# guofei-tju/MVML-MPI

Measured on AMD Instinct MI355X. Metric: molecules/sec GAT-view fwd+bwd at 1/2/4/8 GPU; % HBM peak on aggregation, higher is better.
Workload: dtype f32

## Files before the change

### include/mvml_gat.h

```cpp
#ifndef MVML_GAT_H
#define MVML_GAT_H

#include <stddef.h>
#include <stdint.h>

#ifdef __cplusplus
extern "C" {
#endif

#define MVML_OK 0
#define MVML_ERR_INVALID 1
#define MVML_ERR_LAUNCH 2
#define MVML_ERR_WORKSPACE 3

const char* mvml_last_error(void);
const char* mvml_version(void);

#define MVML_OPT_BIG_WINDOW 0
#define MVML_OPT_BWD_ATOMWISE 1
#define MVML_OPT_GEMM_TILE 2
#define MVML_OPT_GEMM_PERSIST 3
#define MVML_OPT_GEMM_NSPLIT 4
#define MVML_OPT_GEMM_RING 5
#define MVML_OPT_LSTM_TILE 6
// ... 118 lines not shown
                           int64_t ldgx, void* stream);
int mvml_gat_fold_weights(const float* fc_w, const float* res_fc_w, const float* attn_lr, int H,
                          int F, int Fin, int ldw, int mean_residual, float* Wcat, void* stream);
int mvml_gat_unfold_grads(const float* gWcat, const float* attn_lr, int H, int F, int Fin,
                          int ldg, int mean_residual, float* g_fc_w, float* g_res_fc_w,
                          void* stream);
size_t mvml_gat_proj_fwd_workspace_size(int64_t num_nodes, int H, int F);
int mvml_gat_proj_fwd(int64_t num_nodes, const float* X, int64_t ldx, int64_t K,
                      const float* Wcat, int64_t ldw, const float* attn_lr, int H, int F,
                      int mean_residual, int algo , float* Y, int64_t ldy,
                      float* elr, const uint32_t* amax_x, const uint32_t* amax_w,
                      const uint16_t* w_planes, int64_t w_plane, void* workspace,
                      size_t workspace_bytes, void* stream);
size_t mvml_gat_attn_grad_workspace_size(int64_t num_nodes, int H, int F);
int mvml_gat_attn_grad(int64_t num_nodes, int H, int F, const float* Y, int64_t ldy,
                       const float* gelr, int64_t ldgl, float* g_attn_l, float* g_attn_r,
                       void* workspace, size_t workspace_bytes, void* stream);
int mvml_gat_agg_fwd(int64_t num_nodes, const int32_t* node_groups, int64_t num_groups,
                     const int32_t* in_rowptr, const int32_t* in_src, const float* Y, int64_t ldy,
                     int H, int F, const float* elr, const float* bias, float slope, int mode,
                     float* out, float* attn, uint32_t* out_amax, uint32_t* out_row_amax,
                     void* stream);
int mvml_gat_agg_fwd_res(int64_t num_nodes, const int32_t* node_groups, int64_t num_groups,
                         const int32_t* in_rowptr, const int32_t* in_src, const float* Y,
                         int64_t ldy, int H, int F, const float* elr, const float* R, int64_t ldr,
                         const float* bias, float slope, int mode, float* out, float* attn,
                         uint32_t* out_amax, uint32_t* out_row_amax, void* stream);
size_t mvml_gat_agg_bwd_workspace_size(int64_t num_edges, int H);
int mvml_gat_agg_bwd(int64_t num_nodes, const int32_t* node_groups, int64_t num_groups,
                     const int32_t* in_rowptr, const int32_t* in_src, const int32_t* out_rowptr,
                     const int32_t* out_dst, const int32_t* out_inslot, const float* Y,
                     int64_t ldy, const float* elr, const float* attn, const float* out,
                     const float* g_out, int H, int F, float slope, int mode, float* gY,
                     int64_t ldgy, uint32_t* gy_amax, uint32_t* gy_row_amax, void* workspace,
                     size_t workspace_bytes, void* stream);
int mvml_gat_agg_bwd_res(int64_t num_nodes, const int32_t* node_groups, int64_t num_groups,
                         const int32_t* in_rowptr, const int32_t* in_src, const int32_t* out_rowptr,
                         const int32_t* out_dst, const int32_t* out_inslot, const float* Y,
                         int64_t ldy, const float* elr, const float* attn, const float* out,
                         const float* g_out, int H, int F, float slope, int mode, float* gY,
                         int64_t ldgy, int64_t elr_col, float* gR, int64_t ldgr, uint32_t* gy_amax,
                         uint32_t* gy_row_amax, void* workspace, size_t workspace_bytes, void* stream);
size_t mvml_gat_layer_bwd_workspace_size(int64_t num_nodes, int64_t num_edges, int H, int F, int Fin,
                                         int mean);
int mvml_gat_layer_bwd(int64_t num_nodes, const int32_t* node_groups, int64_t num_groups,
                       const int32_t* in_rowptr, const int32_t* in_src, const int32_t* out_rowptr,
                       const int32_t* out_dst, const int32_t* out_inslot, int64_t num_edges, int H,
                       int F, int Fin, int mean, float slope, const float* X, const float* Wcat,
                       const float* attn_lr, const float* Y, int64_t ldy, const float* elr,
                       const float* attn, const float* out, const float* g_out, float* g_X,
                       float* g_fc, float* g_res, float* g_attn, float* g_bias, void* workspace,
                       size_t workspace_bytes, void* stream);

int mvml_gatv2_agg_fwd(int64_t num_nodes, const int32_t* in_rowptr, const int32_t* in_src,
                       const float* ZL, int64_t ldzl, const float* ZR, int64_t ldzr, int H, int F,
                       const float* attn_vec, const float* R, int64_t ldr, float slope, int mode,
                       float* out, float* attn, void* stream);
int64_t mvml_gatv2_partial_rows(int64_t num_nodes);
size_t mvml_gatv2_agg_bwd_workspace_size(int64_t num_nodes, int64_t num_edges, int H, int F);
int mvml_gatv2_agg_bwd(int64_t num_nodes, const int32_t* in_rowptr, const int32_t* in_src,
                       const int32_t* out_rowptr, const int32_t* out_dst, const int32_t* out_inslot,
                       int64_t num_edges, const float* ZL, int64_t ldzl, const float* ZR,
                       int64_t ldzr, int H, int F, const float* attn_vec, const float* attn,
                       const float* out, const float* g_out, float slope, int mode, float* gZL,
                       int64_t ldgzl, float* gZR, int64_t ldgzr, float* gR, int64_t ldgr,
                       float* g_attn_vec, void* workspace, size_t workspace_bytes, void* stream);
int mvml_add_cols_f32(int64_t rows, int cols, const float* src, int64_t lds, float* dst, int64_t ldd,
                      void* stream);

int mvml_lstm_gates_cell_plan_ok(int64_t M, int D, int64_t K);
int mvml_lstm_gates_cell_fwd(int64_t M, int D, int64_t K, const float* A, int64_t lda,
                             const float* w_perm, int64_t ldw, const float* b_ih,
                             const float* b_hh, const float* c_prev, float* c_out, float* h_out,
                             int64_t ldh, float* act, float* h_out2, int64_t ldh2,
                             const uint32_t* amax_a, const uint32_t* amax_b ,
                             const uint32_t* amax_a_rows ,
                             const uint16_t* w_planes, int64_t w_plane ,
                             void* stream);
int mvml_segment_max_bits(int64_t B, const int64_t* node_offsets, const uint32_t* in_bits,
                          uint32_t floor_bits, uint32_t* out_bits, void* stream);
int mvml_lstm_cell_fwd(int64_t B, int D, const float* gates_pre, const float* b_ih,
                       const float* b_hh, const float* c_prev, float* c_out, float* h_out,
                       int64_t ldh, float* act_out, float* h_out2, int64_t ldh2, void* stream);
int64_t mvml_lstm_cell_bwd_part_rows(int64_t B, int D);
int mvml_lstm_cell_bwd(int64_t B, int D, const float* act, const float* c, const float* c_prev,
                       const float* g_h, int64_t ldgh, const float* g_h2, int64_t ldgh2,
                       const float* g_c, float* g_gates, float* g_c_prev, uint32_t* gg_amax,
                       float* gb_part, void* stream);
int mvml_set2set_seg_fwd(int64_t B, int D, const int64_t* node_offsets, const float* X,
                         float* qstar, int64_t ldq, float* lse, void* stream);
int mvml_set2set_seg_bwd(int64_t B, int D, const int64_t* node_offsets, const float* X,
                         const float* qstar, int64_t ldq, const float* lse,
                         const float* g_qstar, int64_t ldgq, float* g_q, int64_t ldgout,
                         float* alpha, float* g_e, void* stream);
int mvml_set2set_gx(int64_t num_nodes, int D, int T, const int32_t* node_graph,
                    const int64_t* node_offsets, int64_t num_graphs,
                    const float* qstars, int64_t ldq, int64_t qstar_stride,
                    const float* g_qstars, int64_t ldgq, int64_t g_qstar_stride,
                    const float* alphas, const float* g_es, float* gX, void* stream);

int mvml_wsum_max_fwd(int64_t B, int64_t N, int D, const int64_t* node_offsets, const float* X,
                      int64_t ldx, const float* W, const float* bias, float* out, int64_t ldo,
                      float* gate, int32_t* argmax, int64_t lda, void* stream);
int64_t mvml_wsum_max_bwd_part_rows(int64_t B);
int mvml_wsum_max_bwd(int64_t B, int64_t N, int D, const int64_t* node_offsets, const float* X,
                      int64_t ldx, const float* W, const float* gate, const int32_t* argmax,
                      int64_t lda, const float* g_out, int64_t ldgo, float* gX, int64_t ldgx,
                      float* part, int64_t ldp, void* stream);

int mvml_graphnorm_fwd(int64_t G, int D, const int64_t* group_offsets, const float* x,
                       const float* weight, const float* bias, const float* mean_scale,
                       float eps, float* y, void* stream);
size_t mvml_graphnorm_bwd_workspace_size(int64_t G, int D);
int mvml_graphnorm_bwd(int64_t G, int D, const int64_t* group_offsets, const float* x,
                       const float* weight, const float* mean_scale, float eps,
                       const float* g_y, float* g_x, float* g_weight, float* g_bias,
                       float* g_mean_scale, void* workspace, size_t workspace_bytes,
                       void* stream);

int64_t mvml_batchnorm1d_part_rows(int64_t M);
size_t mvml_batchnorm1d_workspace_size(int64_t M, int C);
int mvml_batchnorm1d_fwd(int64_t M, int C, const float* x, int64_t ldx, const float* weight,
                         const float* bias, int training, double momentum, double eps,
                         float* running_mean, float* running_var, int64_t* num_batches_tracked,
                         float* y, int64_t ldy, double* save_mean, double* save_invstd,
                         void* workspace, size_t workspace_bytes, void* stream);
int mvml_batchnorm1d_bwd(int64_t M, int C, const float* x, int64_t ldx, const float* weight,
                         int training, const double* save_mean, const double* save_invstd,
                         const float* g_y, int64_t ldgy, float* g_x, int64_t ldgx, float* g_weight,
                         float* g_bias, void* workspace, size_t workspace_bytes, void* stream);

int mvml_relu_bwd(int64_t n, const float* y, const float* g_y, float* g_x, float scale, void* stream);
int mvml_dropout_fwd(int64_t n, const float* x, float* y, double p, int64_t seed, void* stream);
int mvml_copy_cols(int64_t rows, int cols, const float* src, int64_t lds, float* dst, int64_t ldd,
                   void* stream);
int mvml_fill_zero(void* p, int64_t rows, int64_t row_bytes, int64_t pitch_bytes, void* stream);
int mvml_lstm_pack_weights(int D, int kin, const float* w_ih, const float* w_hh, float* wcat,
                           float* wperm, void* stream);
int mvml_transpose(int64_t rows, int64_t cols, const float* src, int64_t lds, float* dst, int64_t ldd,
                   void* stream);
int mvml_scale_by(int64_t n, const float* x, const float* s, float* y, void* stream);

int mvml_layernorm_fwd(int64_t rows, int D, const float* x, int64_t ldx, const float* gamma,
                       const float* beta, float eps, float* y, int64_t ldy, float* mean,
                       float* rstd, void* stream);
int mvml_layernorm_bwd(int64_t rows, int D, const float* x, int64_t ldx, const float* gamma,
                       const float* mean, const float* rstd, const float* g_y, int64_t ldgy,
                       float* g_x, int64_t ldgx, float* g_y_xhat, void* stream);
int mvml_token_attn_fwd(int64_t B, int H, int dk, const float* qkv, int64_t ld, float scale,
                        float* att, float* P, void* stream);
int mvml_token_attn_bwd(int64_t B, int H, int dk, const float* qkv, int64_t ld, float scale,
                        const float* P, const float* g_att, float* g_qkv, int64_t ldg,
                        void* stream);
int mvml_token_attn_fold_fwd(int64_t B, int H, int dk, const float* pv, int64_t ld,
                             const float* x, int64_t ldx, float scale, float* att, float* P,
                             void* stream);
int mvml_token_attn_fold_bwd(int64_t B, int H, int dk, const float* pv, int64_t ld,
                             const float* x, int64_t ldx, float scale, const float* P,
                             const float* g_att, float* g_pv, int64_t ldg, float* g_k,
                             int64_t ldgk, uint32_t* g_pv_amax, void* stream);
int mvml_conv3_fwd(int64_t B, int C, int O, int W, const float* in, const float* weight,
                   const float* bias, float* out, void* stream);
size_t mvml_conv3_bwd_workspace_size(int64_t B);
int mvml_conv3_bwd(int64_t B, int C, int O, int W, const float* in, const float* weight,
                   const float* out, const float* g_out, float* g_in, float* g_weight,
                   float* g_bias, void* workspace, size_t workspace_bytes, void* stream);
// ... 92 lines not shown
```

### mvml-mpi_amd/csrc/capi.cpp

```cpp
#include <stdarg.h>
#include <stdio.h>
#include <stdlib.h>

#include <atomic>

#include "common.h"

namespace mvml {

static thread_local char g_err[512] = {0};

void set_error(const char* fmt, ...) {
  va_list ap;
  va_start(ap, fmt);
  vsnprintf(g_err, sizeof(g_err), fmt, ap);
  va_end(ap);
}

void clear_error() { g_err[0] = 0; }

int check_launch(const char* what) {
  hipError_t e = hipGetLastError();
  if (e != hipSuccess) {
    set_error("%s: %s", what, hipGetErrorString(e));
    return MVML_ERR_LAUNCH;
  }
  return MVML_OK;
}

constexpr int kOptCount = 12;
static std::atomic<int> g_opt[kOptCount];
static int env_int(const char* name, int dflt) {
  const char* e = getenv(name);
  return e ? atoi(e) : dflt;
}
static const bool g_opt_init = [] {
  g_opt[MVML_OPT_BIG_WINDOW] = env_int("MVML_BIG_WINDOW", 1);
  g_opt[MVML_OPT_BWD_ATOMWISE] = env_int("MVML_BWD_ATOMWISE", 0);
  g_opt[MVML_OPT_GEMM_TILE] = env_int("MVML_X3_TILE", 0);
  g_opt[MVML_OPT_GEMM_PERSIST] = env_int("MVML_X3W_PERSIST", 256);
  g_opt[MVML_OPT_GEMM_NSPLIT] = env_int("MVML_GEMM_NSPLIT", 1);
  g_opt[MVML_OPT_GEMM_RING] = env_int("MVML_GEMM_RING", 0);
  g_opt[MVML_OPT_LSTM_TILE] = env_int("MVML_LSTM_TILE", 0);
  g_opt[MVML_OPT_MEAN_SRC] = env_int("MVML_MEAN_SRC", 1);
  g_opt[MVML_OPT_FLAT_SRC] = env_int("MVML_FLAT_SRC", 0);
  g_opt[MVML_OPT_DST_FWD] = env_int("MVML_DST_FWD", 0);
  g_opt[MVML_OPT_DST_UNR] = env_int("MVML_DST_UNR", 0);
  g_opt[MVML_OPT_SMALLK] = env_int("MVML_SMALLK", 1);
  return true;
}();

int option(int i) { return g_opt[i].load(std::memory_order_relaxed); }

}

extern "C" int mvml_set_option(int opt, int value) {
  if (opt < 0 || opt >= mvml::kOptCount) return -1;
  return mvml::g_opt[opt].exchange(value, std::memory_order_relaxed);
}

extern "C" int mvml_get_option(int opt) {
  if (opt < 0 || opt >= mvml::kOptCount) return -1;
  return mvml::option(opt);
}

extern "C" const char* mvml_last_error(void) { return mvml::g_err; }

extern "C" const char* mvml_version(void) { return "mvml_gat 0.1.0 (gfx950)"; }
```

### mvml-mpi_amd/csrc/set2set.hip

```cpp
#include <numeric>

#include "common.h"
#include "wave_ops.h"

namespace mvml {
namespace {

__device__ __forceinline__ float sigm(float x) { return 1.f / (1.f + expf(-x)); }

__global__ void lstm_cell_fwd_kernel(int64_t B, int D, const float* __restrict__ gp,
                                     const float* __restrict__ b_ih, const float* __restrict__ b_hh,
                                     const float* __restrict__ c_prev, float* __restrict__ c_out,
                                     float* __restrict__ h_out, int64_t ldh, float* __restrict__ act,
                                     float* __restrict__ h_out2, int64_t ldh2) {
  const int64_t total = B * D;
  for (int64_t e = (int64_t)blockIdx.x * blockDim.x + threadIdx.x; e < total;
       e += (int64_t)gridDim.x * blockDim.x) {
    const int64_t b = e / D;
    const int d = (int)(e - b * D);
    const float* g = gp ? gp + b * 4 * D : nullptr;
    const float gi = (g ? g[d] : 0.f) + b_ih[d] + b_hh[d];
    const float gf = (g ? g[D + d] : 0.f) + b_ih[D + d] + b_hh[D + d];
    const float gg = (g ? g[2 * D + d] : 0.f) + b_ih[2 * D + d] + b_hh[2 * D + d];
    const float go = (g ? g[3 * D + d] : 0.f) + b_ih[3 * D + d] + b_hh[3 * D + d];
    const float i = sigm(gi), f = sigm(gf), gt = tanhf(gg), o = sigm(go);
    const float cp = c_prev ? c_prev[e] : 0.f;
    const float c = __fmaf_rn(f, cp, __fmul_rn(i, gt));
    c_out[e] = c;
    const float h = __fmul_rn(o, tanhf(c));
    h_out[b * ldh + d] = h;
    if (h_out2) h_out2[b * ldh2 + d] = h;
    float* a = act + b * 4 * D;
    a[d] = i;
    a[D + d] = f;
    a[2 * D + d] = gt;
    a[3 * D + d] = o;
  }
}

__global__ void lstm_cell_bwd_kernel(int64_t B, int D, const float* __restrict__ act,
                                     const float* __restrict__ c, const float* __restrict__ c_prev,
                                     const float* __restrict__ g_h, int64_t ldgh,
                                     const float* __restrict__ g_h2, int64_t ldgh2,
                                     const float* __restrict__ g_c, float* __restrict__ g_gates,
                                     float* __restrict__ g_c_prev, uint32_t* __restrict__ gg_amax,
                                     float* __restrict__ gb_part) {
  const int64_t total = B * D;
  float mx = 0.f;
  float sb[4] = {0.f, 0.f, 0.f, 0.f};
  for (int64_t e = (int64_t)blockIdx.x * blockDim.x + threadIdx.x; e < total;
       e += (int64_t)gridDim.x * blockDim.x) {
    const int64_t b = e / D;
    const int d = (int)(e - b * D);
    const float* a = act + b * 4 * D;
    const float i = a[d], f = a[D + d], gt = a[2 * D + d], o = a[3 * D + d];
    const float gh = g_h2 ? g_h[b * ldgh + d] + g_h2[b * ldgh2 + d] : g_h[b * ldgh + d];
    const float tc = tanhf(c[e]);
    const float gc = (g_c ? g_c[e] : 0.f) + gh * o * (1.f - tc * tc);
    const float cp = c_prev ? c_prev[e] : 0.f;
    float* gg = g_gates + b * 4 * D;
    const float g0 = gc * gt * i * (1.f - i), g1 = gc * cp * f * (1.f - f);
    const float g2 = gc * i * (1.f - gt * gt), g3 = gh * tc * o * (1.f - o);
    gg[d] = g0;
    gg[D + d] = g1;
    gg[2 * D + d] = g2;
    gg[3 * D + d] = g3;
    mx = fmaxf(mx, fmaxf(fmaxf(fabsf(g0), fabsf(g1)), fmaxf(fabsf(g2), fabsf(g3))));
    if (g_c_prev) g_c_prev[e] = gc * f;
    sb[0] += g0;
    sb[1] += g1;
    sb[2] += g2;
    sb[3] += g3;
  }
  if (gb_part) {
    const int64_t gid = (int64_t)blockIdx.x * blockDim.x + threadIdx.x;
    const int64_t r0 = gid / D, d = gid - r0 * D;
    float* pr = gb_part + r0 * 4 * D + d;
#pragma unroll
    for (int q = 0; q < 4; ++q) pr[q * D] = sb[q];
  }
  if (gg_amax) {
    mx = wave_max(mx);
    __shared__ float red[4];
    if ((threadIdx.x & 63) == 0) red[threadIdx.x >> 6] = mx;
    __syncthreads();
    if (threadIdx.x == 0)
      atomicMax(gg_amax, __float_as_uint(fmaxf(fmaxf(red[0], red[1]), fmaxf(red[2], red[3]))));
  }
}

template <int NV>
__global__ void __launch_bounds__(256)
seg_fwd_kernel(int64_t B, int D, const int64_t* __restrict__ node_off, const float* __restrict__ X,
               float* __restrict__ qstar, int64_t ldq, float* __restrict__ lse) {
  const int lane = threadIdx.x & 63;
  const int64_t g = (int64_t)blockIdx.x * 4 + (threadIdx.x >> 6);
  if (g >= B) return;
  const int64_t n0 = node_off[g], n1 = node_off[g + 1];
  float4 q[NV], r[NV];
  bool ok[NV];
#pragma unroll
  for (int c = 0; c < NV; ++c) {
    const int col = 4 * (lane + 64 * c);
    ok[c] = col < D;
    q[c] = ok[c] ? ld4(qstar + g * ldq + col) : make_float4(0, 0, 0, 0);
    r[c] = make_float4(0, 0, 0, 0);
  }
  float m = -INFINITY, s = 0.f;
  for (int64_t n = n0; n < n1; ++n) {
    float4 x[NV];
    float part = 0.f;
#pragma unroll
    for (int c = 0; c < NV; ++c) {
      x[c] = ok[c] ? ld4(X + n * D + 4 * (lane + 64 * c)) : make_float4(0, 0, 0, 0);
      part += dot4_contract(x[c], q[c]);
    }
    const float e = wave_sum(part);
    const float mn = fmaxf(m, e);
    const float sc = expf(m - mn);
// ... 149 lines not shown
    const int cnt = (int)min<int64_t>(64, n1 - base);
    for (int i = 0; i < cnt; ++i) {
      float4 acc[NV];
#pragma unroll
      for (int c = 0; c < NV; ++c) acc[c] = make_float4(0, 0, 0, 0);
#pragma unroll
      for (int t = 0; t < kGxT; ++t) {
        if (t >= T) break;
        const float a_ = __int_as_float(__builtin_amdgcn_readlane(__float_as_int(al[t]), i));
        const float e_ = __int_as_float(__builtin_amdgcn_readlane(__float_as_int(ge[t]), i));
#pragma unroll
        for (int c = 0; c < NV; ++c) {
          const float4 a = gv[t][c], b = qv[t][c];
          acc[c].x += a_ * a.x + e_ * b.x;
          acc[c].y += a_ * a.y + e_ * b.y;
          acc[c].z += a_ * a.z + e_ * b.z;
          acc[c].w += a_ * a.w + e_ * b.w;
        }
      }
#pragma unroll
      for (int c = 0; c < NV; ++c) {
        const int col = 4 * (lane + 64 * c);
        if (col < D) st4(gX + (base + i) * D + col, acc[c]);
      }
    }
  }
}

__global__ void __launch_bounds__(256) segment_max_bits_kernel(int64_t B, const int64_t* __restrict__ offs,
                                                               const uint32_t* __restrict__ in,
                                                               uint32_t floor_bits, uint32_t* __restrict__ out) {
  for (int64_t b = (int64_t)blockIdx.x * 256 + threadIdx.x; b < B; b += (int64_t)gridDim.x * 256) {
    uint32_t m = floor_bits;
    for (int64_t n = offs[b]; n < offs[b + 1]; ++n) m = max(m, in[n]);
    out[b] = m;
  }
}

unsigned grid_for(int64_t total) {
  return (unsigned)std::max<int64_t>(1, std::min<int64_t>(ceil_div(total, 256), 16384));
}

int check_d(int D, const char* who) {
  MVML_REQUIRE(D > 0 && D % 4 == 0 && D <= 1024, "%s: feature size must be a multiple of 4 <= 1024 (got %d)", who, D);
  return MVML_OK;
}

}
}

using namespace mvml;

#define MVML_NV_SWITCH(KERNEL, GRID, ...)                                                   \
  switch ((int)ceil_div(D, 256)) {                                                          \
    case 1: KERNEL<1><<<GRID, 256, 0, st>>>(__VA_ARGS__); break;                            \
    case 2: KERNEL<2><<<GRID, 256, 0, st>>>(__VA_ARGS__); break;                            \
    case 3: KERNEL<3><<<GRID, 256, 0, st>>>(__VA_ARGS__); break;                            \
    default: KERNEL<4><<<GRID, 256, 0, st>>>(__VA_ARGS__); break;                           \
  }

extern "C" int mvml_segment_max_bits(int64_t B, const int64_t* node_offsets, const uint32_t* in_bits,
                                     uint32_t floor_bits, uint32_t* out_bits, void* stream) {
  clear_error();
  MVML_REQUIRE(B >= 0 && (B == 0 || (node_offsets && in_bits && out_bits)), "segment_max_bits: bad args");
  if (B == 0) return MVML_OK;
  hipStream_t st = as_stream(stream);
  segment_max_bits_kernel<<<grid_for(B), 256, 0, st>>>(B, node_offsets, in_bits, floor_bits, out_bits);
  return check_launch("segment_max_bits_kernel");
}

extern "C" int mvml_lstm_cell_fwd(int64_t B, int D, const float* gates_pre, const float* b_ih,
                                  const float* b_hh, const float* c_prev, float* c_out,
                                  float* h_out, int64_t ldh, float* act_out, float* h_out2,
                                  int64_t ldh2, void* stream) {
  clear_error();
  MVML_REQUIRE(B >= 0 && D > 0 && ldh >= D && (!h_out2 || ldh2 >= D), "lstm_cell_fwd: bad shape");
  if (B == 0) return MVML_OK;
  hipStream_t st = as_stream(stream);
  lstm_cell_fwd_kernel<<<grid_for(B * D), 256, 0, st>>>(B, D, gates_pre, b_ih, b_hh, c_prev, c_out,
                                                        h_out, ldh, act_out, h_out2, ldh2);
  return check_launch("lstm_cell_fwd_kernel");
}

static int64_t cell_bwd_part_rows(int64_t B, int D) {
  const int64_t step = 256 / std::gcd<int64_t>(D, 256);
  return std::max<int64_t>(step, ceil_div(ceil_div(B, 16), step) * step);
}
extern "C" int64_t mvml_lstm_cell_bwd_part_rows(int64_t B, int D) {
  return (B > 0 && D > 0) ? cell_bwd_part_rows(B, D) : 0;
}

extern "C" int mvml_lstm_cell_bwd(int64_t B, int D, const float* act, const float* c,
                                  const float* c_prev, const float* g_h, int64_t ldgh,
                                  const float* g_h2, int64_t ldgh2,
                                  const float* g_c, float* g_gates, float* g_c_prev,
                                  uint32_t* gg_amax, float* gb_part, void* stream) {
  clear_error();
  MVML_REQUIRE(B >= 0 && D > 0 && ldgh >= D && (!g_h2 || ldgh2 >= D), "lstm_cell_bwd: bad shape");
  if (B == 0) return MVML_OK;
  hipStream_t st = as_stream(stream);
  if (gb_part) {
    const int64_t R = cell_bwd_part_rows(B, D);
    lstm_cell_bwd_kernel<<<(unsigned)(R * D / 256), 256, 0, st>>>(B, D, act, c, c_prev, g_h, ldgh,
                                                                  g_h2, ldgh2, g_c, g_gates, g_c_prev,
                                                                  gg_amax, gb_part);
    return check_launch("lstm_cell_bwd_kernel");
  }
  const unsigned grid = gg_amax ? (unsigned)std::min<int64_t>(
                                      grid_for(B * D), std::max<int64_t>(256, ceil_div(B * D, 4096)))
                                : grid_for(B * D);
  lstm_cell_bwd_kernel<<<grid, 256, 0, st>>>(B, D, act, c, c_prev, g_h, ldgh, g_h2, ldgh2, g_c,
                                             g_gates, g_c_prev, gg_amax, nullptr);
  return check_launch("lstm_cell_bwd_kernel");
}

extern "C" int mvml_set2set_seg_fwd(int64_t B, int D, const int64_t* node_offsets, const float* X,
                                    float* qstar, int64_t ldq, float* lse, void* stream) {
  clear_error();
  int rc = check_d(D, "set2set_seg_fwd");
  if (rc) return rc;
  MVML_REQUIRE(ldq >= 2 * D && ldq % 4 == 0, "set2set_seg_fwd: bad ldq");
  if (B == 0) return MVML_OK;
  hipStream_t st = as_stream(stream);
  const unsigned grid = (unsigned)ceil_div(B, 4);
  MVML_NV_SWITCH(seg_fwd_kernel, grid, B, D, node_offsets, X, qstar, ldq, lse)
  return check_launch("seg_fwd_kernel");
}

extern "C" int mvml_set2set_seg_bwd(int64_t B, int D, const int64_t* node_offsets, const float* X,
                                    const float* qstar, int64_t ldq, const float* lse,
                                    const float* g_qstar, int64_t ldgq, float* g_q,
                                    int64_t ldgout, float* alpha, float* g_e, void* stream) {
  clear_error();
  int rc = check_d(D, "set2set_seg_bwd");
  if (rc) return rc;
  MVML_REQUIRE(ldq >= 2 * D && ldgq >= 2 * D && ldgout >= D, "set2set_seg_bwd: bad ld");
  if (B == 0) return MVML_OK;
  hipStream_t st = as_stream(stream);
  const unsigned grid = (unsigned)ceil_div(B, 4);
  MVML_NV_SWITCH(seg_bwd_kernel, grid, B, D, node_offsets, X, qstar, ldq, lse, g_qstar, ldgq, g_q,
                 ldgout, alpha, g_e)
  return check_launch("seg_bwd_kernel");
}

extern "C" int mvml_set2set_gx(int64_t num_nodes, int D, int T, const int32_t* node_graph,
                               const int64_t* node_offsets, int64_t num_graphs,
                               const float* qstars, int64_t ldq, int64_t qstar_stride,
                               const float* g_qstars, int64_t ldgq, int64_t g_qstar_stride,
                               const float* alphas, const float* g_es, float* gX, void* stream) {
  clear_error();
  int rc = check_d(D, "set2set_gx");
  if (rc) return rc;
  MVML_REQUIRE(T >= 0 && ldq >= 2 * D && ldgq >= 2 * D, "set2set_gx: bad shape");
  if (num_nodes == 0) return MVML_OK;
  hipStream_t st = as_stream(stream);
  if (node_offsets && num_graphs > 0 && T <= kGxT && D <= 512) {
    const unsigned grid = (unsigned)ceil_div(num_graphs, 4);
    if (D <= 256)
      seg_gx_mol_kernel<1><<<grid, 256, 0, st>>>(num_graphs, D, T, node_offsets, qstars, ldq,
                                                 qstar_stride, g_qstars, ldgq, g_qstar_stride,
                                                 alphas, g_es, num_nodes, gX);
    else
      seg_gx_mol_kernel<2><<<grid, 256, 0, st>>>(num_graphs, D, T, node_offsets, qstars, ldq,
                                                 qstar_stride, g_qstars, ldgq, g_qstar_stride,
                                                 alphas, g_es, num_nodes, gX);
    return check_launch("seg_gx_mol_kernel");
// ... 8 lines not shown
```

### mvml-mpi_amd/mvml_gat/__init__.py

```python
from ._lib import MvmlError, lib
from .batching import BatchedMolGraph, MolGraph, batch, bigraph_from_bonds, from_arrays, graph
from .fusion import FPNModule, MVFusion, bce_with_logits
from .smiles import RNNModule, collate_smiles, tokens_struct
from .nn import GAT, GATConv, GATLayer, GATv2, GATv2Conv, GATv2Layer, GNNModule, GraphNorm, Set2Set, WeightAndSum, WeightedSumAndMax
from .nn import GATPredictor, GATv2Predictor, MLPPredictor
from .optim import FlatAdam
from .mvp import MVP
from .metrics import MultiLabelMeter, evaluate, evaluate_class_wise

__all__ = ["MultiLabelMeter", "evaluate", "evaluate_class_wise","GNNModule", "MVFusion", "FPNModule", "RNNModule", "tokens_struct", "collate_smiles", "bce_with_logits", "GAT", "GATLayer", "GATConv", "GATv2", "GATv2Layer", "GATv2Conv", "Set2Set", "WeightAndSum", "WeightedSumAndMax", "GATPredictor", "GATv2Predictor", "MLPPredictor", "GraphNorm", "BatchedMolGraph",
           "MolGraph", "batch", "graph", "bigraph_from_bonds", "from_arrays", "lib", "MvmlError", "FlatAdam", "MVP"]
__version__ = "0.1.0"
```

### mvml-mpi_amd/mvml_gat/functional.py

```python
import contextlib
import ctypes
import os

import numpy as np
import torch

from . import _lib
from ._lib import call, ptr

MODE_FLATTEN_ELU, MODE_MEAN, MODE_FLATTEN = 0, 1, 2
RES_PROJ, RES_IDENTITY, RES_NONE = "proj", "identity", "none"
_MVML_RES_NONE = 2


def _check_cuda_f32(t, name):
    if not t.is_cuda:
        raise RuntimeError(f"{name} must be a CUDA (HIP) tensor: the mvml_gat path has no CPU fallback")
    if t.dtype != torch.float32:
        raise TypeError(f"{name} must be float32, got {t.dtype}")


def _c(t):
    return t if t.is_contiguous() else t.contiguous()

# ... 465 lines not shown
        if sep:
            call("mvml_gat_unfold_grads_res", ptr(gW), ptr(attn_lr), H, F, Fin, Fp, _MVML_RES_NONE,
                 ptr(g_fc), None, st)
        else:
            g_res = torch.empty((HF, Fin), dtype=torch.float32, device=dev)
            call("mvml_gat_unfold_grads", ptr(gW), ptr(attn_lr), H, F, Fin, Fp, mean_res, ptr(g_fc),
                 ptr(g_res), st)
        gelr = gY[:, C:CE]
        g_alr = torch.empty((2, HF), dtype=torch.float32, device=dev)
        gemm_batched(gW[C:], Wcat, 2, F, Fp, 0, 0, H * Fp, Fp, g_alr, HF, H, Fp, F * Fp, F)
        g_al = g_alr[0].view_as(attn_l)
        g_ar = g_alr[1].view_as(attn_r)
        if DEBUG_CAPTURE is not None:
            DEBUG_CAPTURE.update(elr=elr, gelr=gelr, attn=attn)
        if has_bias and mean_res:
            if sep:
                colsum(g_out, N, F, F, g_bias, alpha=1.0 / H)
            elif not bias_done:
                colsum(gY, N, F, ldg, g_bias, offset=HF, alpha=1.0 / H)
            if H > 1:
                copy2d(g_bias.view(H, F)[1:], g_bias[:F].view(1, F).expand(H - 1, F))
        elif has_bias and sep:
            colsum(gR, N, HF, ldgr, g_bias)
        elif has_bias and not bias_done:
            colsum(gY, N, HF, ldg, g_bias, offset=HF)
        if ctx.needs_input_grad[0]:
            beta = 1.0 if res_kind == RES_IDENTITY else 0.0
            if gX is None:
                gX = torch.empty((N, Fin), dtype=torch.float32, device=dev)
                if beta:
                    call("mvml_head_mean_bwd_f32", N, H, F, ptr(g_out), F, ptr(gX), Fin, st)
            link = ctx.elu_claim
            if link is not None and amx is not None and ROW_SCALES and ctx.wil is not None:
                zero_(link.amax)
                _lib.call_tag[0] = {"flops": 2 * N * Fin * CE, "shape": (N, Fin, CE, 0, 1)}
                call("mvml_gemm_f16x2_ex", N, Fin, CE, 1, ptr(gY), ldg, 0, ptr(Wcat), Fp, 1, ptr(ctx.wil),
                     0, ptr(gyr if gyr is not None else absmax_rows(gY, N, CE, ldg)), 0, slot(amx, 1),
                     None, 0, 3, ptr(gX), Fin, 0, ptr(Xp), Fp, ptr(link.amax), None, 0, 0, 0, st)
                link.g_rst = gX
            elif amx is not None and ROW_SCALES:
                gemm(gY, Wcat, N, Fin, CE, 0, 1, ldg, Fp, gX, Fin, amax=(None, slot(amx, 1)),
                     arows=gyr if gyr is not None else absmax_rows(gY, N, CE, ldg), bil4=ctx.wil, beta=beta)
            else:
                gemm(gY, Wcat, N, Fin, CE, 0, 1, ldg, Fp, gX, Fin, algo=ctx.algo,
                     amax=None if amx is None else (slot(amx, 2), slot(amx, 1)), beta=beta)
        else:
            gX = None
        return gX, g_fc, g_res, g_al, g_ar, g_bias, None, None, None, None, None, None, None


COLSUM_FUSED = os.environ.get("MVML_COLSUM_FUSED", "1") != "0"


CELL_EPI = True


class Set2SetFunction(torch.autograd.Function):

    @staticmethod
    def forward(ctx, X, g, n_iters, n_layers, *lstm_params):
        _check_cuda_f32(X, "feat")
        X = _c(X)
        N, D = X.shape
        B = g.batch_size
        dev = X.device
        st = _stream(dev)
        T, Lr = n_iters, n_layers
        W = [tuple(_c(p) for p in lstm_params[4 * l:4 * l + 4]) for l in range(Lr)]
        f32 = dict(dtype=torch.float32, device=dev)
        kin = [2 * D] + [D] * (Lr - 1)
        XH = [torch.empty((T + 1, B, kin[l] + D), **f32) for l in range(Lr)]
        zero_(XH[0][0])
        for l in range(1, Lr):
            zero_(XH[l][0, :, D:])
        L = _lib.lib()
        Wcat = [torch.empty((4 * D, kin[l] + D), **f32) for l in range(Lr)]
        Wperm = [torch.empty((4 * D, kin[l] + D), **f32) if CELL_EPI else None for l in range(Lr)]
        for l in range(Lr):
            call("mvml_lstm_pack_weights", D, kin[l], ptr(W[l][0]), ptr(W[l][1]), ptr(Wcat[l]), ptr(Wperm[l]), st)
        acts = torch.empty((T, Lr, B, 4 * D), **f32)
        cs = torch.empty((T, Lr, B, D), **f32)
        lse = torch.empty((T, B), **f32)
        gates = torch.empty((B, 4 * D), **f32)
        amax_x = amax_w = None
        mrows = None
        wsp = [(None, 0)] * Lr
        if GEMM_ALGO == "f16x2":
            kx = known_amax(X)
            if kx is None:
                kx = (zeros(1, dtype=torch.int32, device=dev), 0)
                absmax(X, N, D, D, kx[0], 0, accumulate=True)
            amax_x = torch.empty(1, dtype=torch.int32, device=dev)
            call("mvml_segment_max_bits", 1, ptr(_unit_segment(dev)), slot(*kx), 0x3F800000, ptr(amax_x), st)
            if ROW_SCALES:
                xr = row_maxima(X, N, D, D)
                mrows = torch.empty(max(B, 1), dtype=torch.int32, device=dev)
                call("mvml_segment_max_bits", B, ptr(g.node_offsets), ptr(xr), 0x3F800000, ptr(mrows), st)
            amax_w = torch.empty(Lr, dtype=torch.int32, device=dev)
            for l in range(Lr):
                absmax(Wcat[l], 4 * D, kin[l] + D, kin[l] + D, amax_w, l)
            wsp = [(split_il4(Wperm[l] if CELL_EPI else Wcat[l], 4 * D, kin[l] + D, kin[l] + D,
                              slot(amax_w, l)), 0) for l in range(Lr)]
        for t in range(T):
            for l in range(Lr):
                w_ih, w_hh, b_ih, b_hh = W[l]
                K = kin[l] + D if t > 0 else kin[l]
                own = XH[l][t + 1][:, kin[l]:]
                nxt = XH[l + 1][t] if l < Lr - 1 else XH[0][t + 1]
                c_prev = cs[t - 1, l] if t > 0 else None
                ldn = kin[l + 1] + D if l < Lr - 1 else 3 * D
                if CELL_EPI and not (t == 0 and l == 0) and L.mvml_lstm_gates_cell_plan_ok(B, D, K):
                    pa = pw = None
                    if amax_x is not None:
                        pa, pw = slot(amax_x, 0), slot(amax_w, l)
                    _lib.call_tag[0] = {"flops": 2 * B * 4 * D * K, "shape": (B, 4 * D, K, 0, 0, "cell")}
                    call("mvml_lstm_gates_cell_fwd", B, D, K, ptr(XH[l][t]), kin[l] + D, ptr(Wperm[l]),
                         kin[l] + D, ptr(b_ih), ptr(b_hh), ptr(c_prev), ptr(cs[t, l]), ptr(own),
                         kin[l] + D, ptr(acts[t, l]), ptr(nxt), ldn, pa, pw, ptr(mrows),
                         ptr(wsp[l][0]), wsp[l][1], st)
                    continue
                gp = gates
                if t == 0 and l == 0:
                    gp = None
                else:
                    gemm(XH[l][t], Wcat[l], B, 4 * D, K, 0, 0, kin[l] + D, kin[l] + D, gates, 4 * D,
                         amax=None if amax_x is None else (slot(amax_x, 0), slot(amax_w, l)),
                         arows=mrows,
                         bil4=wsp[l][0] if not CELL_EPI and wsp[l][1] == 0 else None)
                call("mvml_lstm_cell_fwd", B, D, ptr(gp), ptr(b_ih), ptr(b_hh), ptr(c_prev),
                     ptr(cs[t, l]), ptr(own), kin[l] + D, ptr(acts[t, l]), ptr(nxt), ldn, st)
            call("mvml_set2set_seg_fwd", B, D, ptr(g.node_offsets), ptr(X), ptr(XH[0][t + 1]), 3 * D,
                 ptr(lse[t]), st)
        ctx.save_for_backward(X, acts, cs, lse, *XH, *[p for w in W for p in w])
        ctx.g, ctx.T, ctx.Lr = g, T, Lr
        ctx.amax = (amax_x, amax_w)
        return copy2d(torch.empty((B, 2 * D), **f32), XH[0][T][:, :2 * D])

    @staticmethod
    def backward(ctx, g_out):
        X, acts, cs, lse, *rest = ctx.saved_tensors
        g, T, Lr = ctx.g, ctx.T, ctx.Lr
        XH, flat = rest[:Lr], rest[Lr:]
        W = [tuple(flat[4 * l:4 * l + 4]) for l in range(Lr)]
        qs = XH[0][1:]
        N, D = X.shape
        B = g.batch_size
        dev = X.device
        st = _stream(dev)
        f32 = dict(dtype=torch.float32, device=dev)
        kins = [2 * D] + [D] * (Lr - 1)
        Wcat = [torch.empty((4 * D, kins[l] + D), **f32) for l in range(Lr)]
        for l in range(Lr):
            call("mvml_lstm_pack_weights", D, kins[l], ptr(W[l][0]), ptr(W[l][1]), ptr(Wcat[l]), None, st)
        g_qs3 = torch.empty((T, B, 3 * D), **f32)
        g_qstars = g_qs3[:, :, :2 * D]
        copy2d(g_qstars[T - 1], _c(g_out))
        alphas = torch.empty((T, N), **f32)
        g_es = torch.empty((T, N), **f32)
        gW_ih = [torch.empty_like(w[0]) for w in W]
        gW_hh = [torch.empty_like(w[1]) for w in W]
        gb = [torch.empty_like(w[2]) for w in W]
        g_gates_all = torch.empty((Lr, T, B, 4 * D), **f32)
        g_h = torch.empty((B, D), **f32)
        gxh = [None] + [torch.empty((B, 2 * D), **f32) for _ in range(1, Lr)]
        g_c = [torch.empty((B, D), **f32) for _ in range(Lr)]
        g_c_new = torch.empty((B, D), **f32)
        R = int(_lib.lib().mvml_lstm_cell_bwd_part_rows(B, D))
        gb_part = torch.empty((Lr, T, R, 4 * D), **f32)
        amax_x, amax_w = ctx.amax
        amax_g = zeros(Lr, dtype=torch.int32, device=dev) if amax_x is not None else None
        wib = [None] * Lr
        if amax_g is not None:
            wib = [split_il4(Wcat[l], 4 * D, Wcat[l].shape[1], Wcat[l].shape[1], slot(amax_w, l))
                   for l in range(Lr)]
        for t in range(T - 1, -1, -1):
            call("mvml_set2set_seg_bwd", B, D, ptr(g.node_offsets), ptr(X), ptr(qs[t]), 3 * D,
                 ptr(lse[t]), ptr(g_qs3[t]), 3 * D, ptr(g_h), D, ptr(alphas[t]), ptr(g_es[t]), st)
            for l in range(Lr - 1, -1, -1):
                kin = 2 * D if l == 0 else D
                if l == Lr - 1:
                    gh, ldgh = g_h, D
                else:
                    gh, ldgh = gxh[l + 1][:, :D], 2 * D
                gh2, ldgh2 = None, 0
                if t < T - 1:
                    gh2, ldgh2 = (g_qs3[t][:, 2 * D:], 3 * D) if l == 0 else (gxh[l][:, D:], 2 * D)
                c_prev = cs[t - 1, l] if t > 0 else None
                g_gates = g_gates_all[l, t]
                call("mvml_lstm_cell_bwd", B, D, ptr(acts[t, l]), ptr(cs[t, l]), ptr(c_prev), ptr(gh), ldgh,
                     ptr(gh2), ldgh2,
                     ptr(g_c[l]) if t < T - 1 else None, ptr(g_gates), ptr(g_c_new), slot(amax_g, l),
                     ptr(gb_part[l, t]), st)
                g_c[l], g_c_new = g_c_new, g_c[l]
                ncols = kin + D if t > 0 else (kin if l > 0 else 0)
                if ncols:
                    out, ldo = (g_qs3[t - 1], 3 * D) if l == 0 else (gxh[l], 2 * D)
                    gemm(g_gates, Wcat[l], B, ncols, 4 * D, 0, 1, 4 * D, kin + D, out, ldo,
                         amax=None if amax_g is None else (slot(amax_g, l), slot(amax_w, l)),
                         bil4=wib[l])
        for l in range(Lr):
            G = g_gates_all[l]
            kin = 2 * D if l == 0 else D
            ldx = kin + D
            t0 = 1 if l == 0 else 0
            if T > t0:
                gWcat = torch.empty((4 * D, ldx), **f32)
                gemm(G[t0:], XH[l][t0:T], 4 * D, ldx, (T - t0) * B, 1, 1, 4 * D, ldx, gWcat, ldx,
                     amax=None if amax_g is None else (slot(amax_g, l), slot(amax_x, 0)))
                copy2d(gW_ih[l], gWcat[:, :kin])
                copy2d(gW_hh[l], gWcat[:, kin:])
            else:
                zero_(gW_ih[l])
                zero_(gW_hh[l])
            colsum(gb_part[l], T * R, 4 * D, 4 * D, gb[l])
        gX = torch.empty((N, D), **f32)
        call("mvml_set2set_gx", N, D, T, ptr(g.node_graph), ptr(g.node_offsets), B, ptr(qs), 3 * D, B * 3 * D,
             ptr(g_qs3), 3 * D, B * 3 * D, ptr(alphas), ptr(g_es), ptr(gX), st)
        grads = []
        for l in range(Lr):
            grads += [gW_ih[l], gW_hh[l], gb[l], copy2d(torch.empty_like(gb[l]), gb[l])]
        return (gX, None, None, None, *grads)


def _rows_f32(t):
    if t.dim() == 2 and t.stride(1) == 1 and t.stride(0) % 4 == 0 and t.stride(0) >= t.shape[1] \
            and t.data_ptr() % 16 == 0:
        return t
    return t.contiguous()


class WeightedSumAndMaxFunction(torch.autograd.Function):

    @staticmethod
    def forward(ctx, X, weight, bias, g):
        _check_cuda_f32(X, "feats")
        X = _rows_f32(X)
        N, D = X.shape
        B = g.batch_size
        dev = X.device
        weight, bias = _c(weight), _c(bias)
        out = torch.empty((B, 2 * D), dtype=torch.float32, device=dev)
        gate = torch.empty(N, dtype=torch.float32, device=dev)
        argmax = torch.empty((B, D), dtype=torch.int32, device=dev)
        if B == 0 or N == 0:
            if B:
                zero_(out)
                argmax.fill_(-1)
        else:
            call("mvml_wsum_max_fwd", B, N, D, ptr(g.node_offsets), ptr(X), X.stride(0), ptr(weight),
                 ptr(bias), ptr(out), 2 * D, ptr(gate), ptr(argmax), D, _stream(dev))
        if DEBUG_CAPTURE is not None:
            DEBUG_CAPTURE.setdefault("readout_argmax", []).append(argmax.detach().clone())
        ctx.save_for_backward(X, weight, gate, argmax)
        ctx.g = g
        return out

    @staticmethod
    def backward(ctx, g_out):
        X, weight, gate, argmax = ctx.saved_tensors
        g = ctx.g
        N, D = X.shape
        B = g.batch_size
        dev = X.device
        g_out = _rows_f32(g_out)
        gX = torch.empty((N, D), dtype=torch.float32, device=dev)
        gW = torch.empty((1, D), dtype=torch.float32, device=dev)
        gb = torch.empty(1, dtype=torch.float32, device=dev)
        if B == 0 or N == 0:
            return gX, zero_(gW), zero_(gb), None
        R = _lib.lib().mvml_wsum_max_bwd_part_rows(B)
        ldp = D + 4
        part = torch.empty((R, ldp), dtype=torch.float32, device=dev)
        call("mvml_wsum_max_bwd", B, N, D, ptr(g.node_offsets), ptr(X), X.stride(0), ptr(weight),
             ptr(gate), ptr(argmax), D, ptr(g_out), g_out.stride(0), ptr(gX), D, ptr(part), ldp,
             _stream(dev))
        colsum(part, R, D, ldp, gW)
        colsum(part, R, 1, ldp, gb, offset=D)
        return gX, gW, gb, None


class GraphNormFunction(torch.autograd.Function):

    @staticmethod
    def forward(ctx, x, weight, bias, mean_scale, group_offsets, eps):
        _check_cuda_f32(x, "x")
        x = _c(x)
        G = group_offsets.numel() - 1
        D = x.shape[1]
        y = torch.empty_like(x)
        call("mvml_graphnorm_fwd", G, D, ptr(group_offsets), ptr(x), ptr(_c(weight)), ptr(_c(bias)),
             ptr(_c(mean_scale)), float(eps), ptr(y), _stream(x.device))
        ctx.save_for_backward(x, weight, mean_scale, group_offsets)
        ctx.eps = eps
        return y

# ... 398 lines not shown
```

Baseline: 468,300.

## Exploit batch-uniform first LSTM step in upper Set2Set layers via broadcast and rank-1 grads

At t=0 for layers above the first, the input row is the same for every graph in the batch (it derives from a zero initial state), so the gate GEMM is replaced by a single-row matvec plus a broadcast kernel that writes c, h and the activations for all B rows. In the backward pass the t=0 weight gradient is computed as a rank-1 update (column sum of the gate gradients times the shared input row) instead of being folded into the large GEMM over all timesteps. This removes one B-row GEMM per upper layer in forward and shrinks the K dimension of the weight-gradient GEMM, at the cost of extra small kernel launches and an assumption that XH[l][0] rows are identical across the batch.

```diff
diff --git a/include/mvml_gat.h b/include/mvml_gat.h
--- a/include/mvml_gat.h
+++ b/include/mvml_gat.h
@@ -224,6 +224,12 @@
 int mvml_lstm_cell_fwd(int64_t B, int D, const float* gates_pre, const float* b_ih,
                        const float* b_hh, const float* c_prev, float* c_out, float* h_out,
                        int64_t ldh, float* act_out, float* h_out2, int64_t ldh2, void* stream);
+int mvml_lstm_cell0_bcast_fwd(int64_t B, int D, int64_t K, const float* x, const float* w_ih,
+                              int64_t ldw, const float* b_ih, const float* b_hh, float* row,
+                              float* c_out, float* h_out, int64_t ldh, float* act_out,
+                              float* h_out2, int64_t ldh2, void* stream);
+int mvml_rank1_add_f32(int64_t M, int64_t N, const float* u, const float* v, float beta, float* C,
+                       int64_t ldc, void* stream);
 int64_t mvml_lstm_cell_bwd_part_rows(int64_t B, int D);
 int mvml_lstm_cell_bwd(int64_t B, int D, const float* act, const float* c, const float* c_prev,
                        const float* g_h, int64_t ldgh, const float* g_h2, int64_t ldgh2,
diff --git a/mvml-mpi_amd/csrc/capi.cpp b/mvml-mpi_amd/csrc/capi.cpp
--- a/mvml-mpi_amd/csrc/capi.cpp
+++ b/mvml-mpi_amd/csrc/capi.cpp
@@ -66,4 +66,4 @@
 
 extern "C" const char* mvml_last_error(void) { return mvml::g_err; }
 
-extern "C" const char* mvml_version(void) { return "mvml_gat 0.1.0 (gfx950)"; }
+extern "C" const char* mvml_version(void) { return "mvml_gat 0.2.0 (gfx950)"; }
diff --git a/mvml-mpi_amd/csrc/set2set.hip b/mvml-mpi_amd/csrc/set2set.hip
--- a/mvml-mpi_amd/csrc/set2set.hip
+++ b/mvml-mpi_amd/csrc/set2set.hip
@@ -35,6 +35,66 @@
     a[D + d] = f;
     a[2 * D + d] = gt;
     a[3 * D + d] = o;
+  }
+}
+
+__global__ void __launch_bounds__(256)
+lstm_cell0_row_kernel(int D, int K, const float* __restrict__ x, const float* __restrict__ w_ih,
+                      int64_t ldw, const float* __restrict__ b_ih, const float* __restrict__ b_hh,
+                      float* __restrict__ row) {
+  const int lane = threadIdx.x & 63;
+  const int d = blockIdx.x * 4 + (threadIdx.x >> 6);
+  if (d >= D) return;
+  float pre[4];
+#pragma unroll
+  for (int q = 0; q < 4; ++q) {
+    const float* w = w_ih + (int64_t)(q * D + d) * ldw;
+    float s = 0.f;
+    for (int k = lane; k < K; k += 64) s = __fmaf_rn(w[k], x[k], s);
+    pre[q] = wave_sum(s) + b_ih[q * D + d] + b_hh[q * D + d];
+  }
+  if (lane == 0) {
+    const float i = sigm(pre[0]), f = sigm(pre[1]), gt = tanhf(pre[2]), o = sigm(pre[3]);
+    const float c = __fmaf_rn(f, 0.f, __fmul_rn(i, gt));
+    row[d] = c;
+    row[D + d] = __fmul_rn(o, tanhf(c));
+    row[2 * D + d] = i;
+    row[3 * D + d] = f;
+    row[4 * D + d] = gt;
+    row[5 * D + d] = o;
+  }
+}
+
+__global__ void __launch_bounds__(256)
+lstm_cell0_bcast_kernel(int64_t B, int D, const float* __restrict__ row, float* __restrict__ c_out,
+                        float* __restrict__ h_out, int64_t ldh, float* __restrict__ act,
+                        float* __restrict__ h_out2, int64_t ldh2) {
+  const int D4 = D / 4;
+  const int64_t total = B * D4;
+  for (int64_t e = (int64_t)blockIdx.x * blockDim.x + threadIdx.x; e < total;
+       e += (int64_t)gridDim.x * blockDim.x) {
+    const int64_t b = e / D4;
+    const int d = 4 * (int)(e - b * D4);
+    st4(c_out + b * D + d, ld4(row + d));
+    const float4 h = ld4(row + D + d);
+    st4(h_out + b * ldh + d, h);
+    if (h_out2) st4(h_out2 + b * ldh2 + d, h);
+    float* a = act + b * 4 * D + d;
+#pragma unroll
+    for (int q = 0; q < 4; ++q) st4(a + q * D, ld4(row + (2 + q) * D + d));
+  }
+}
+
+__global__ void __launch_bounds__(256)
+rank1_add_kernel(int64_t M, int64_t N, const float* __restrict__ u, const float* __restrict__ v,
+                 float beta, float* __restrict__ C, int64_t ldc) {
+  const int64_t total = M * N;
+  for (int64_t e = (int64_t)blockIdx.x * blockDim.x + threadIdx.x; e < total;
+       e += (int64_t)gridDim.x * blockDim.x) {
+    const int64_t i = e / N, j = e - i * N;
+    float* c = C + i * ldc + j;
+    const float p = __fmul_rn(u[i], v[j]);
+    *c = beta == 0.f ? p : __fmaf_rn(beta, *c, p);
   }
 }
 
@@ -350,6 +410,39 @@
   return check_launch("lstm_cell_fwd_kernel");
 }
 
+extern "C" int mvml_lstm_cell0_bcast_fwd(int64_t B, int D, int64_t K, const float* x,
+                                         const float* w_ih, int64_t ldw, const float* b_ih,
+                                         const float* b_hh, float* row, float* c_out, float* h_out,
+                                         int64_t ldh, float* act_out, float* h_out2, int64_t ldh2,
+                                         void* stream) {
+  clear_error();
+  int rc = check_d(D, "lstm_cell0_bcast_fwd");
+  if (rc) return rc;
+  MVML_REQUIRE(B >= 0 && K > 0 && K < (int64_t(1) << 30) && ldw >= K, "lstm_cell0_bcast_fwd: bad shape");
+  if (B == 0) return MVML_OK;
+  MVML_REQUIRE(x && w_ih && b_ih && b_hh, "lstm_cell0_bcast_fwd: null input");
+  MVML_REQUIRE(row && aligned16(row) && c_out && aligned16(c_out) && act_out && aligned16(act_out) &&
+                   row_ok(h_out, ldh, D) && (!h_out2 || row_ok(h_out2, ldh2, D)),
+               "lstm_cell0_bcast_fwd: outputs must be 16-B aligned with row strides that are multiples of 4");
+  hipStream_t st = as_stream(stream);
+  lstm_cell0_row_kernel<<<(unsigned)ceil_div(D, 4), 256, 0, st>>>(D, (int)K, x, w_ih, ldw, b_ih, b_hh, row);
+  rc = check_launch("lstm_cell0_row_kernel");
+  if (rc) return rc;
+  lstm_cell0_bcast_kernel<<<grid_for(B * (D / 4)), 256, 0, st>>>(B, D, row, c_out, h_out, ldh, act_out,
+                                                                 h_out2, ldh2);
+  return check_launch("lstm_cell0_bcast_kernel");
+}
+
+extern "C" int mvml_rank1_add_f32(int64_t M, int64_t N, const float* u, const float* v, float beta,
+                                  float* C, int64_t ldc, void* stream) {
+  clear_error();
+  MVML_REQUIRE(M >= 0 && N >= 0 && ldc >= N, "rank1_add_f32: bad shape");
+  if (M == 0 || N == 0) return MVML_OK;
+  MVML_REQUIRE(u && v && C, "rank1_add_f32: null pointer");
+  rank1_add_kernel<<<grid_for(M * N), 256, 0, as_stream(stream)>>>(M, N, u, v, beta, C, ldc);
+  return check_launch("rank1_add_kernel");
+}
+
 static int64_t cell_bwd_part_rows(int64_t B, int D) {
   const int64_t step = 256 / std::gcd<int64_t>(D, 256);
   return std::max<int64_t>(step, ceil_div(ceil_div(B, 16), step) * step);
diff --git a/mvml-mpi_amd/mvml_gat/__init__.py b/mvml-mpi_amd/mvml_gat/__init__.py
--- a/mvml-mpi_amd/mvml_gat/__init__.py
+++ b/mvml-mpi_amd/mvml_gat/__init__.py
@@ -10,4 +10,4 @@
 
 __all__ = ["MultiLabelMeter", "evaluate", "evaluate_class_wise","GNNModule", "MVFusion", "FPNModule", "RNNModule", "tokens_struct", "collate_smiles", "bce_with_logits", "GAT", "GATLayer", "GATConv", "GATv2", "GATv2Layer", "GATv2Conv", "Set2Set", "WeightAndSum", "WeightedSumAndMax", "GATPredictor", "GATv2Predictor", "MLPPredictor", "GraphNorm", "BatchedMolGraph",
            "MolGraph", "batch", "graph", "bigraph_from_bonds", "from_arrays", "lib", "MvmlError", "FlatAdam", "MVP"]
-__version__ = "0.1.0"
+__version__ = "0.2.0"
diff --git a/mvml-mpi_amd/mvml_gat/functional.py b/mvml-mpi_amd/mvml_gat/functional.py
--- a/mvml-mpi_amd/mvml_gat/functional.py
+++ b/mvml-mpi_amd/mvml_gat/functional.py
@@ -571,6 +571,7 @@
         cs = torch.empty((T, Lr, B, D), **f32)
         lse = torch.empty((T, B), **f32)
         gates = torch.empty((B, 4 * D), **f32)
+        row0 = torch.empty(6 * D, **f32)
         amax_x = amax_w = None
         mrows = None
         wsp = [(None, 0)] * Lr
@@ -598,6 +599,11 @@
                 nxt = XH[l + 1][t] if l < Lr - 1 else XH[0][t + 1]
                 c_prev = cs[t - 1, l] if t > 0 else None
                 ldn = kin[l + 1] + D if l < Lr - 1 else 3 * D
+                if t == 0 and l > 0:
+                    call("mvml_lstm_cell0_bcast_fwd", B, D, kin[l], ptr(XH[l][0]), ptr(w_ih), kin[l],
+                         ptr(b_ih), ptr(b_hh), ptr(row0), ptr(cs[0, l]), ptr(own),
+                         kin[l] + D, ptr(acts[0, l]), ptr(nxt), ldn, st)
+                    continue
                 if CELL_EPI and not (t == 0 and l == 0) and L.mvml_lstm_gates_cell_plan_ok(B, D, K):
                     pa = pw = None
                     if amax_x is not None:
@@ -691,15 +697,23 @@
             G = g_gates_all[l]
             kin = 2 * D if l == 0 else D
             ldx = kin + D
-            t0 = 1 if l == 0 else 0
-            if T > t0:
+            u0 = None
+            if l > 0 and B > 0:
+                u0 = torch.empty(4 * D, **f32)
+                colsum(gb_part[l, 0], R, 4 * D, 4 * D, u0)
+            if T > 1:
                 gWcat = torch.empty((4 * D, ldx), **f32)
-                gemm(G[t0:], XH[l][t0:T], 4 * D, ldx, (T - t0) * B, 1, 1, 4 * D, ldx, gWcat, ldx,
+                gemm(G[1:], XH[l][1:T], 4 * D, ldx, (T - 1) * B, 1, 1, 4 * D, ldx, gWcat, ldx,
                      amax=None if amax_g is None else (slot(amax_g, l), slot(amax_x, 0)))
+                if u0 is not None:
+                    call("mvml_rank1_add_f32", 4 * D, kin, ptr(u0), ptr(XH[l][0]), 1.0, ptr(gWcat), ldx, st)
                 copy2d(gW_ih[l], gWcat[:, :kin])
                 copy2d(gW_hh[l], gWcat[:, kin:])
             else:
-                zero_(gW_ih[l])
+                if u0 is not None:
+                    call("mvml_rank1_add_f32", 4 * D, kin, ptr(u0), ptr(XH[l][0]), 0.0, ptr(gW_ih[l]), kin, st)
+                else:
+                    zero_(gW_ih[l])
                 zero_(gW_hh[l])
             colsum(gb_part[l], T * R, 4 * D, 4 * D, gb[l])
         gX = torch.empty((N, D), **f32)
```

New measurement: 472,500 (median of 6 runs). No clear change (+0.9%).
